# Changfei-Fu/RUMI-SLAM

Measured on AMD Instinct MI355X. Metric: frames/sec ORB extract+match, higher is better.
Workload: dtype u8; 1 GPU; ORB extract (640x480, 8-level pyramid, 1000 features/frame) + brute-force 256-bit Hamming match of consecutive frames (BASELINE.json configs[1]+[2]); scaling=n/a (one GPU), exchange=none

## Files before the change

### rumi_slam_amd/csrc/orb_kernels.hip

```cpp
#include <hip/hip_runtime.h>

#include "orb_device.h"
#include "orb_math.h"

namespace rumi {

struct PatternF { float v[256 * 4]; };
constexpr PatternF make_pattern_f() {
    constexpr int8_t src[256 * 4] = {
#include "orb_pattern.inc"
    };
    PatternF p{};
    for (int i = 0; i < 256 * 4; i++) p.v[i] = (float)src[i];
    return p;
}
__constant__ PatternF c_patternF = make_pattern_f();

__device__ __forceinline__ unsigned xcd_swizzle(unsigned lin, unsigned total) {
    const unsigned q = total >> 3, r = total & 7, xcd = lin & 7;
    return (xcd < r ? xcd * (q + 1) : r * (q + 1) + (xcd - r) * q) + (lin >> 3);
}

struct __attribute__((packed)) U32 { uint32_t v; };
struct __attribute__((packed)) U64 { uint64_t v; };
// ... 367 lines not shown
    const uint32_t to = (g[1] | g[2]) & (g[5] | g[6]), uo = (g[3] | g[4]) & (g[7] | g[0]);
    return (te | ue) & (to | uo);
}
__device__ __forceinline__ uint32_t fast_bytes_ringmask(uint32_t y, uint32_t z) {
    const uint32_t f = ((y & 0x80808080u) | (~(z >> 1) & 0x40404040u));
    return f * 0x41041u;
}

template <int CTP>
__device__ __forceinline__ int fast_score_cell_bytes(const uint8_t *tile, uint8_t *sc, uint16_t *cl, uint16_t *sl, int tp, int dw, int dh, int tlow, int lane) {
    const int TP = CTP ? CTP : tp;
    const int ng = (dw + 7) >> 3;
    const int nItems = ng * dh;
    const unsigned Mng = magic_of(ng);
    const int scDelta = -2 * TP - 3;
    const uint32_t mLast = 0xFFFFu >> (2 * (8 * ng - dw));
    const uint32_t TT = (uint32_t)tlow * 0x01000100u;
    uint32_t *cl32 = reinterpret_cast<uint32_t *>(cl);
    int pending = 0, nScored = 0;
    auto drain = [&]() {
        int head = 0;
        while (pending >= 128) {
            wave_lds_fence();
            fast_score_batch<CTP>(tile, sc, sl, nScored, cl + head, 128, tp, scDelta, tlow, lane);
            head += 128;
            pending -= 128;
        }
        if (head) {
            wave_lds_fence();
            const uint32_t q = cl32[(head >> 1) + lane];
            wave_lds_fence();
            if (2 * lane < pending) cl32[lane] = q;
        }
    };
    for (int base = 0; base < nItems; base += 64) {
        const int ip = base + lane;
        const bool live = ip < nItems;
        const int row = live ? magic_div(ip, Mng) : 0, gi = live ? ip - mul24(row, ng) : 0;
        const int A = mul24(row + 3, TP) + 8 * gi + 4;
        const uint8_t *t = tile + A;
#define RUMI_DW(off) (*reinterpret_cast<const uint32_t *>(t + (off)))
        const uint32_t M3a = RUMI_DW(-3 * TP), M3b = RUMI_DW(-3 * TP + 4), P3a = RUMI_DW(3 * TP), P3b = RUMI_DW(3 * TP + 4);
        const uint32_t M2l = RUMI_DW(-2 * TP - 4), M2a = RUMI_DW(-2 * TP), M2b = RUMI_DW(-2 * TP + 4), M2r = RUMI_DW(-2 * TP + 8);
        const uint32_t P2l = RUMI_DW(2 * TP - 4), P2a = RUMI_DW(2 * TP), P2b = RUMI_DW(2 * TP + 4), P2r = RUMI_DW(2 * TP + 8);
        const uint32_t Cl = RUMI_DW(-4), Ca = RUMI_DW(0), Cb = RUMI_DW(4), Cr = RUMI_DW(8);
#undef RUMI_DW
        const uint32_t m0 = __builtin_amdgcn_alignbyte(M2a, M2l, 2), m1 = __builtin_amdgcn_alignbyte(M2b, M2a, 2), m2 = __builtin_amdgcn_alignbyte(M2r, M2b, 2);
        const uint32_t p0 = __builtin_amdgcn_alignbyte(P2a, P2l, 2), p1 = __builtin_amdgcn_alignbyte(P2b, P2a, 2), p2 = __builtin_amdgcn_alignbyte(P2r, P2b, 2);
        const uint32_t ra[8] = {P3a, p1, __builtin_amdgcn_alignbyte(Cb, Ca, 3), m1, M3a, m0, __builtin_amdgcn_alignbyte(Ca, Cl, 1), p0};
        const uint32_t rb[8] = {P3b, p2, __builtin_amdgcn_alignbyte(Cr, Cb, 3), m2, M3b, m1, __builtin_amdgcn_alignbyte(Cb, Ca, 1), p1};
        uint32_t nba, nda, nbb, ndb;
        fast_bytes_thresholds(Ca, TT, nba, nda);
        fast_bytes_thresholds(Cb, TT, nbb, ndb);
        uint32_t ba[8], ga[8], bb[8], gb[8];
#pragma unroll
        for (int k = 0; k < 8; k++) {
            ba[k] = __builtin_amdgcn_lerp(ra[k], nba, 0u);
            ga[k] = __builtin_amdgcn_lerp(ra[k], nda, 0x01010101u);
            bb[k] = __builtin_amdgcn_lerp(rb[k], nbb, 0u);
            gb[k] = __builtin_amdgcn_lerp(rb[k], ndb, 0x01010101u);
        }
        uint32_t m = __builtin_amdgcn_perm(fast_bytes_ringmask(four_of_eight(bb), four_of_eight_dual(gb)),
                                           fast_bytes_ringmask(four_of_eight(ba), four_of_eight_dual(ga)), 0x0c0c0703u);
        if (gi == ng - 1) m &= mLast;
        if (!live) m = 0;
        if (__ballot(m != 0) != 0) {
            const int cnt = __popc(m);
            const int incl = wave_incl_scan(cnt);
            const int total = __builtin_amdgcn_readlane(incl, 63);
            auto append = [&](uint16_t *w) {
                for (uint32_t r = m; r; r &= r - 1) {
                    const uint32_t b = __builtin_ctz(r);
                    *w++ = (uint16_t)(((uint32_t)A + (b >> 1)) | ((b & 1u) << 15));
                }
            };
            if (pending + total <= kRingCap) {
                append(cl + pending + incl - cnt);
                pending = __builtin_amdgcn_readfirstlane(pending + total);
                drain();
            } else {
                const int half = __builtin_amdgcn_readlane(incl, 31);
                if (lane < 32) append(cl + pending + incl - cnt);
                pending = __builtin_amdgcn_readfirstlane(pending + half);
                drain();
                if (lane >= 32) append(cl + pending + incl - half - cnt);
                pending = __builtin_amdgcn_readfirstlane(pending + total - half);
                drain();
            }
        }
    }
    wave_lds_fence();
    if (pending) fast_score_batch<CTP>(tile, sc, sl, nScored, cl, pending, tp, scDelta, tlow, lane);
    return nScored;
}

struct FastCell {
    const uint8_t *img;
    long long cellIdx;
    int pitch, rows, cols, nd;
    int ox, oy;
    bool live;
};
__device__ __forceinline__ FastCell fast_cell_geom(const DevParams *__restrict__ P, const ImgSrc &src, int cell, int frame, int32_t *__restrict__ cellCnt, int lane) {
    FastCell g;
    g.live = false;
    if (cell >= P->totalCells) return g;
    int level = 0;
    for (int l = 1; l < P->nlevels; l++)
        if (cell >= P->lv[l].cellBase) level = l;
    const DevLevel &L = P->lv[level];
    const int ci = cell - L.cellBase;
    const int ci_i = ci / L.nCols, ci_j = ci - ci_i * L.nCols;
    g.cellIdx = (long long)frame * P->totalCells + cell;
    const int iniY = kBorder + ci_i * L.hCell, iniX = kBorder + ci_j * L.wCell;
    const int maxY = min(iniY + L.hCell + 6, L.maxBY), maxX = min(iniX + L.wCell + 6, L.maxBX);
    g.cols = maxX - iniX; g.rows = maxY - iniY;
    if (iniY >= L.maxBY - 3 || iniX >= L.maxBX - 6 || g.cols < 7 || g.rows < 7) {
        if (lane == 0) cellCnt[g.cellIdx] = 0;
        return g;
    }
    g.img = level_base(src, P, level, frame, &g.pitch) + (long long)iniY * g.pitch + (iniX - 1);
    g.nd = ((g.cols - 6 + 3) >> 2) + 2;
    g.ox = ci_j * L.wCell; g.oy = ci_i * L.hCell;
    g.live = true;
    return g;
}
constexpr int kStageDepth = 10;
template <int TPC>
__device__ __forceinline__ void fast_cell_stage(const FastCell &g, uint8_t *tile, int tp, int lane) {
    const int TP = TPC ? TPC : tp;
    const int ndT = TP >> 2, rps = min(64 / ndT, 7);
    const int r0 = lane / ndT, c = lane - r0 * ndT;
    if (r0 < rps && c < g.nd) {
        const uint8_t *src = g.img + r0 * g.pitch + 4 * c;
        uint8_t *dst = tile + r0 * TP + 4 * c;
        const int nb = (g.rows + rps - 1) / rps, lastRow = g.rows - rps;
        uint32_t v[kStageDepth];
#pragma unroll
        for (int j = 0; j < kStageDepth; j++)
            if (j < nb) v[j] = reinterpret_cast<const U32 *>(src + (long long)min(j * rps, lastRow) * g.pitch)->v;
#pragma unroll
        for (int j = 0; j < kStageDepth; j++)
            if (j < nb) *reinterpret_cast<uint32_t *>(dst + min(j * rps, lastRow) * TP) = v[j];
        for (int j = kStageDepth; j < nb; j++)
            *reinterpret_cast<uint32_t *>(dst + min(j * rps, lastRow) * TP) = reinterpret_cast<const U32 *>(src + (long long)min(j * rps, lastRow) * g.pitch)->v;
    }
}

template <int TPC>
__device__ __forceinline__ void fast_cell_process(const DevParams *__restrict__ P, const FastLds &F, const FastCell &g, uint8_t *tile, uint8_t *sc,
                                                  uint32_t *__restrict__ cellBuf, int32_t *__restrict__ cellCnt, int lane) {
    const int TP = TPC ? TPC : F.tp;
    const int dw = g.cols - 6, dh = g.rows - 6;
    const unsigned Mdw = magic_of(dw), Mtp = magic_of(TP);
    for (int idx = lane * 16; idx < (dh + 2) * TP; idx += 1024) *reinterpret_cast<uint4 *>(&sc[idx]) = make_uint4(0, 0, 0, 0);
    wave_lds_fence();
    const int npx = dw * dh;
    const int scDelta = -2 * TP - 3;
    uint16_t *cl = reinterpret_cast<uint16_t *>(sc + F.scBytes);
    uint16_t *sl = cl + kRingCap;
    int thr = max(1, P->iniTh);
    uint32_t *out = cellBuf + g.cellIdx * P->maxCellCand;
    int found;
#pragma nounroll
    for (int pass = 0;; pass++) {
        const int nScored = fast_score_cell_bytes<TPC>(tile, sc, cl, sl, TP, dw, dh, thr, lane);
        wave_lds_fence();
        const bool listed = nScored <= kScoredCap;
        const int nItems = listed ? nScored : npx;
        found = 0;
        for (int base = 0; base < nItems; base += 128) {
            int si[2];
            bool in[2];
#pragma unroll
            for (int h = 0; h < 2; h++) {
                const int k = base + 64 * h + lane;
                in[h] = k < nItems;
                if (listed) {
                    si[h] = (int)sl[in[h] ? k : 0] + scDelta;
                } else {
                    const int kk = in[h] ? k : 0, py = magic_div(kk, Mdw);
                    si[h] = mul24(py + 1, TP) + (kk - mul24(py, dw)) + 1;
                }
            }
            int v[2];
            bool isMax[2];
#pragma unroll
            for (int h = 0; h < 2; h++) {
                const uint8_t *s = &sc[si[h]];
                v[h] = s[0];
                const int n0 = s[-TP - 1], n1 = s[-TP], n2 = s[-TP + 1], n3 = s[-1], n4 = s[1], n5 = s[TP - 1], n6 = s[TP], n7 = s[TP + 1];
                isMax[h] = in[h] & (v[h] > 0) & (v[h] > n0) & (v[h] > n1) & (v[h] > n2) & (v[h] > n3) & (v[h] > n4) & (v[h] > n5) & (v[h] > n6) & (v[h] > n7);
            }
            const unsigned long long b0 = __ballot(isMax[0]), b1 = __ballot(isMax[1]);
            const int c0 = __popcll(b0);
#pragma unroll
            for (int h = 0; h < 2; h++) {
                if (isMax[h]) {
                    const unsigned long long b = h ? b1 : b0;
                    const int slot = __builtin_amdgcn_mbcnt_hi((uint32_t)(b >> 32), __builtin_amdgcn_mbcnt_lo((uint32_t)b, found + (h ? c0 : 0)));
                    const int py1 = magic_div(si[h], Mtp), px1 = si[h] - mul24(py1, TP);
                    const uint32_t x = (uint32_t)(px1 + 2 + g.ox), y = (uint32_t)(py1 + 2 + g.oy);
                    out[slot] = x | (y << 12) | ((uint32_t)v[h] << 24);
                }
            }
            found += c0 + __popcll(b1);
        }
        if (found > 0 || pass == 1) break;
        thr = max(1, P->minTh);
    }
    if (lane == 0) cellCnt[g.cellIdx] = found;
}

template <int TPC>
__device__ __forceinline__ void fast_cells_body(const DevParams *__restrict__ P, const ImgSrc &src, const FastLds &F, uint32_t *__restrict__ cellBuf,
                                                int32_t *__restrict__ cellCnt, unsigned bx, unsigned gx) {
    extern __shared__ __attribute__((aligned(16))) uint8_t fl[];
    const int lane = threadIdx.x & 63, wave = __builtin_amdgcn_readfirstlane(threadIdx.x >> 6);
    const unsigned wg = xcd_swizzle(blockIdx.y * gx + bx, gx * gridDim.y);
    const int wpg = blockDim.x >> 6;
    const int cell = (wg % gx) * wpg + wave, frame = wg / gx;
    uint8_t *tile = fl + (size_t)wave * F.perWave;
    uint8_t *sc = tile + F.tileBytes;
    const int TP = TPC ? TPC : F.tp;
    const FastCell gA = fast_cell_geom(P, src, cell, frame, cellCnt, lane);
    if (!gA.live) return;
    fast_cell_stage<TPC>(gA, tile, TP, lane);
    fast_cell_process<TPC>(P, F, gA, tile, sc, cellBuf, cellCnt, lane);
}
template <int TPC>
__global__ __launch_bounds__(256) void k_fast_cells(const DevParams *__restrict__ P, ImgSrc src, FastLds F,
                                                    uint32_t *__restrict__ cellBuf, int32_t *__restrict__ cellCnt) {
    fast_cells_body<TPC>(P, src, F, cellBuf, cellCnt, blockIdx.x, gridDim.x);
}

constexpr int kCompactThreads = 256;
__global__ __launch_bounds__(kCompactThreads) void k_compact(const DevParams *__restrict__ P, const uint32_t *__restrict__ cellBuf,
                                                 const int32_t *__restrict__ cellCnt, uint32_t *__restrict__ cand,
                                                 int32_t *__restrict__ levelStart, int32_t *__restrict__ errFlag) {
    extern __shared__ int sStart[];
    __shared__ int part[kCompactThreads];
    const int tid = threadIdx.x, frame = blockIdx.x;
    const int nc = P->totalCells;
    const int32_t *cnt = cellCnt + (long long)frame * nc;
    const int chunk = (nc + kCompactThreads - 1) / kCompactThreads;
    int sum = 0;
    for (int k = 0; k < chunk; k++) {
        const int c = tid * chunk + k;
        if (c < nc) sum += cnt[c];
    }
    const int lane = tid & 63, wave = __builtin_amdgcn_readfirstlane(tid >> 6);
    int inc = sum;
#pragma unroll
    for (int o = 1; o < 64; o <<= 1) {
        const int t = __shfl_up(inc, o);
        if (lane >= o) inc += t;
    }
    if (lane == 63) part[wave] = inc;
    __syncthreads();
    int base = 0, total = 0;
#pragma unroll
    for (int w = 0; w < kCompactThreads / 64; w++) {
        const int t = part[w];
        if (w < wave) base += t;
        total += t;
    }
    if (tid == 0) sStart[nc] = total;
    int run = base + inc - sum;
    for (int k = 0; k < chunk; k++) {
        const int c = tid * chunk + k;
        if (c < nc) { sStart[c] = run; run += cnt[c]; }
    }
    __syncthreads();
    int32_t *ls = levelStart + (long long)frame * (kMaxLevels + 1);
    if (blockIdx.y == 0 && tid <= P->nlevels) {
        const int c = tid < P->nlevels ? P->lv[tid].cellBase : nc;
        ls[tid] = sStart[c];
    }
    if (blockIdx.y == 0 && tid < P->nlevels) {
        const int c0 = P->lv[tid].cellBase, c1 = c0 + P->lv[tid].nCells;
        if (sStart[c1] - sStart[c0] > P->lv[tid].candCap) atomicOr(errFlag, 16);
    }
    uint32_t *out = cand + (long long)frame * P->totalCand;
    const int nOut = min(sStart[nc], P->totalCand);
    const uint32_t *inBase = cellBuf + (long long)frame * nc * P->maxCellCand;
    for (int j = blockIdx.y * kCompactThreads + tid; j < nOut; j += kCompactThreads * gridDim.y) {
        int lo = 0, hi = nc;
        while (hi - lo > 1) {
            const int mid = (lo + hi) >> 1;
            if (sStart[mid] <= j) lo = mid; else hi = mid;
        }
        out[j] = inBase[(long long)lo * P->maxCellCand + (j - sStart[lo])];
    }
}

constexpr int kBlurRowsSmall = 16, kBlurRowsBatch = 64;

struct BlurGrid { int base[kMaxLevels + 1]; int gx[kMaxLevels]; int bw[kMaxLevels]; };
__device__ __forceinline__ uint32_t mad_u24(uint32_t a, uint32_t b, uint32_t c) {
    uint32_t r;
    asm("v_mad_u32_u24 %0, %1, %2, %3" : "=v"(r) : "v"(a), "v"(b), "v"(c));
    return r;
}
template <int VARIANT, int kBlurRows>
__device__ __forceinline__ void blur_body(const DevParams *__restrict__ P, const ImgSrc &src, const BlurGrid &G, unsigned bxg, unsigned gxg) {
    constexpr uint32_t kT2 = VARIANT ? 49u : 48u, kT3 = VARIANT ? 55u : 56u;
    const int lane = threadIdx.x & 63, wave = __builtin_amdgcn_readfirstlane(threadIdx.x >> 6);
    const unsigned wg = xcd_swizzle(blockIdx.y * gxg + bxg, gxg * gridDim.y);
    const int frame = wg / gxg, lin = wg % gxg;
    int level = 0;
    for (int l = 1; l < P->nlevels; l++)
        if (lin >= G.base[l]) level = l;
    const DevLevel &L = P->lv[level];
    const int bx = (lin - G.base[level]) % G.gx[level], by = (lin - G.base[level]) / G.gx[level];
    const int bw = G.bw[level];
    const int xa = bx * bw + lane * 4;
    const int y0 = (by * 4 + wave) * kBlurRows;
    if (y0 >= L.h) return;
    int pitch;
    const uint8_t *img = level_base(src, P, level, frame, &pitch);
    uint8_t *out = src.blur + (long long)frame * P->arenaStride + L.off;
    const int w = L.w, h = L.h;
    const int xLast = (w - 1) & ~3;
    const int xl = min(xa, xLast);
    const bool firstBlock = bx == 0;
    const bool edgeWave = bx * bw + bw + 4 > w;
    const bool produce = lane * 4 < bw && xa < w;
    uint32_t selA = 0x03020100u, selB = 0x07060504u;
    if (edgeWave && xa + 3 >= w && xa <= xLast + 4) {
#pragma unroll
        for (int i = 0; i < 4; i++) {
            const int x = xa + i;
            if (x < w) continue;
            const int sx = 2 * (w - 1) - x, d = (xa - (sx & ~3)) >> 2;
            const uint32_t a = (d == 1 ? 4u : 0u) + (uint32_t)(sx & 3);
            const uint32_t b = d == 0 ? 4u + (uint32_t)(sx & 3) : (uint32_t)i;
            selA = (selA & ~(0xFFu << (8 * i))) | (a << (8 * i));
            selB = (selB & ~(0xFFu << (8 * i))) | (b << (8 * i));
        }
    }
    int ring[7][4];
#pragma unroll
    for (int k = 0; k < 7; k++)
#pragma unroll
        for (int i = 0; i < 4; i++) ring[k][i] = 0;
    const int yEnd = min(y0 + kBlurRows, h), rEnd = yEnd + 3;
    uint8_t *orow = out + (long long)(y0 - 6) * L.pitch + xa - L.pitch;
    const int haloOff = lane == 0 ? (firstBlock ? 0 : -4) : (lane == 63 && !edgeWave && bw == 256 ? 4 : 0);
    uint32_t Cn[7], Hn[7];
    auto fetch = [&](int r, uint32_t &C, uint32_t &H) {
        const int rc = min(r, rEnd - 1);
        const int rr = rc < 0 ? -rc : (rc >= h ? 2 * (h - 1) - rc : rc);
        const uint8_t *row = img + (long long)rr * pitch + xl;
        C = *reinterpret_cast<const uint32_t *>(row);
        H = 0;
        if (haloOff) H = *reinterpret_cast<const uint32_t *>(row + haloOff);
    };
#pragma unroll
    for (int j = 0; j < 7; j++) fetch(y0 - 3 + j, Cn[j], Hn[j]);
    uint32_t Cm[7], Hm[7];
    auto walk7 = [&](const uint32_t (&Cc)[7], const uint32_t (&Hc)[7], int r0) {
#pragma unroll
        for (int j = 0; j < 7; j++) {
            const int r = r0 + j;
            if (r >= rEnd) break;
            orow += L.pitch;
            uint32_t C = Cc[j];
            if (edgeWave) {
                const uint32_t c1 = __shfl_up(C, 1), c2 = __shfl_up(c1, 1);
                C = __builtin_amdgcn_perm(C, __builtin_amdgcn_perm(c1, c2, selA), selB);
            }
            uint32_t Lw = __shfl_up(C, 1), Rw = __shfl_down(C, 1);
            if (lane == 0) Lw = firstBlock ? __builtin_amdgcn_perm(C, C, 0x01020300u) : Hc[j];
            if (lane == 63 && !edgeWave && bw == 256) Rw = Hc[j];
            constexpr uint32_t tA = 18u | (34u << 8) | (kT2 << 16) | (kT3 << 24), tB = kT2 | (34u << 8) | (18u << 16);
            const uint32_t A0 = __builtin_amdgcn_alignbyte(C, Lw, 1), A1 = __builtin_amdgcn_alignbyte(C, Lw, 2), A2 = __builtin_amdgcn_alignbyte(C, Lw, 3);
            const uint32_t B0 = __builtin_amdgcn_alignbyte(Rw, C, 1), B1 = __builtin_amdgcn_alignbyte(Rw, C, 2), B2 = __builtin_amdgcn_alignbyte(Rw, C, 3);
            ring[j][0] = (int)__builtin_amdgcn_udot4(B0, tB, __builtin_amdgcn_udot4(A0, tA, 0u, false), false);
            ring[j][1] = (int)__builtin_amdgcn_udot4(B1, tB, __builtin_amdgcn_udot4(A1, tA, 0u, false), false);
            ring[j][2] = (int)__builtin_amdgcn_udot4(B2, tB, __builtin_amdgcn_udot4(A2, tA, 0u, false), false);
            ring[j][3] = (int)__builtin_amdgcn_udot4(Rw, tB, __builtin_amdgcn_udot4(C, tA, 0u, false), false);
            const int y = r - 3;
            if (y >= y0 && produce) {
                uint32_t o[4];
#pragma unroll
                for (int i = 0; i < 4; i++) {
                    uint32_t acc = mad_u24(kT3, (uint32_t)ring[(j + 4) % 7][i], 32768u);
                    acc = mad_u24(kT2, (uint32_t)(ring[(j + 3) % 7][i] + ring[(j + 5) % 7][i]), acc);
                    acc = mad_u24(34u, (uint32_t)(ring[(j + 2) % 7][i] + ring[(j + 6) % 7][i]), acc);
                    acc = mad_u24(18u, (uint32_t)(ring[(j + 1) % 7][i] + ring[j][i]), acc);
                    if (VARIANT) acc = min(acc, 0x00FFFFFFu);
                    o[i] = acc;
                }
                const uint32_t p01 = __builtin_amdgcn_perm(o[1], o[0], 0x0c0c0602u), p23 = __builtin_amdgcn_perm(o[3], o[2], 0x06020c0cu);
                *reinterpret_cast<uint32_t *>(orow) = p01 | p23;
            }
        }
    };
    for (int r0 = y0 - 3; r0 < rEnd; r0 += 7) {
#pragma unroll
        for (int j = 0; j < 7; j++) Cm[j] = Cn[j], Hm[j] = Hn[j];
        if (r0 + 7 < rEnd) {
#pragma unroll
            for (int j = 0; j < 7; j++) fetch(r0 + 7 + j, Cn[j], Hn[j]);
        }
        walk7(Cm, Hm, r0);
    }
}
template <int VARIANT, int kBlurRows>
__global__ __launch_bounds__(256) void k_blur(const DevParams *__restrict__ P, ImgSrc src, BlurGrid G) {
    blur_body<VARIANT, kBlurRows>(P, src, G, blockIdx.x, gridDim.x);
}
template <int TPC, int VARIANT>
__global__ __launch_bounds__(256) void k_fast_blur(const DevParams *__restrict__ P, ImgSrc src, FastLds F, uint32_t *__restrict__ cellBuf,
                                                   int32_t *__restrict__ cellCnt, BlurGrid G, unsigned gxFast) {
    if (blockIdx.x < gxFast) fast_cells_body<TPC>(P, src, F, cellBuf, cellCnt, blockIdx.x, gxFast);
    else blur_body<VARIANT, kBlurRowsSmall>(P, src, G, blockIdx.x - gxFast, gridDim.x - gxFast);
}

__device__ __forceinline__ int half_wave_sum(int v) {
    v += __builtin_amdgcn_update_dpp(0, v, 0x111, 0xF, 0xF, false);
    v += __builtin_amdgcn_update_dpp(0, v, 0x112, 0xF, 0xF, false);
    v += __builtin_amdgcn_update_dpp(0, v, 0x114, 0xF, 0xF, false);
    v += __builtin_amdgcn_update_dpp(0, v, 0x118, 0xF, 0xF, false);
    v += __builtin_amdgcn_update_dpp(0, v, 0x142, 0xA, 0xF, false);
    const int lo = __builtin_amdgcn_readlane(v, 31), hi = __builtin_amdgcn_readlane(v, 63);
    return (threadIdx.x & 32) ? hi : lo;
}
__device__ __forceinline__ int wave_sum(int v) {
#pragma unroll
    for (int o = 32; o > 0; o >>= 1) v += __shfl_xor(v, o);
    return v;
}

constexpr int kDiscP = 48, kPatchP = 48;
constexpr int kKpPerWg = 8;

struct AssembleArgs {
    const uint32_t *selLevel; const int32_t *selLevelCnt; int selLevelCap, lap0, lap1;
    int32_t *counts; long long countsStride; int32_t *errFlag, *errMirror;
    uint32_t *selPackedOut, *selMetaOut; int32_t *selCountOut;
};
template <int kKpGroups, bool kAssemble>
__global__ __launch_bounds__(256, 7) void k_orient_desc(const DevParams *__restrict__ P, ImgSrc src,
                                                     const uint32_t *__restrict__ selPacked,
                                                     const uint32_t *__restrict__ selMeta,
                                                     const int32_t *__restrict__ selCount, int selCap,
                                                     RumiKeyPoint *__restrict__ kpOut, long long kpStride, uint8_t *__restrict__ descOut,
                                                     long long descStride, int outCap, AssembleArgs A) {
    static_assert(kDiscP == kPatchP, "the disc and the patch share their rows");
    __shared__ __attribute__((aligned(16))) uint8_t sWin[kKpPerWg][37 * kPatchP];
    __shared__ __attribute__((aligned(16))) float sPat[256 * 4];
    __shared__ int4 sLv[kMaxLevels];
    __shared__ float2 sLvF[kMaxLevels];
    reinterpret_cast<float4 *>(sPat)[threadIdx.x] = reinterpret_cast<const float4 *>(c_patternF.v)[threadIdx.x];
    if (threadIdx.x < (unsigned)P->nlevels) {
        const DevLevel &Lv = P->lv[threadIdx.x];
        sLv[threadIdx.x] = threadIdx.x == 0 ? make_int4(0, src.l0Pitch, (int)Lv.off, Lv.pitch) : make_int4((int)Lv.off, Lv.pitch, (int)Lv.off, Lv.pitch);
        sLvF[threadIdx.x] = make_float2(Lv.scale, Lv.patchSize);
    }
    const int lane = threadIdx.x & 31, hw = threadIdx.x >> 5;
    const unsigned wg = xcd_swizzle(blockIdx.y * gridDim.x + blockIdx.x, gridDim.x * gridDim.y);
    const int kb = (wg % gridDim.x) * (kKpPerWg * kKpGroups) + hw, frame = wg / gridDim.x;
    int cnt;
    __shared__ uint32_t sOwnPk[kAssemble ? kKpPerWg * kKpGroups : 1], sOwnMt[kAssemble ? kKpPerWg * kKpGroups : 1];
    if constexpr (!kAssemble) {
        cnt = selCount[frame];
        __syncthreads();
    } else {
        __shared__ int sLvStart[kMaxLevels + 1], sRed[2], sOwnF[kKpPerWg * kKpGroups];
        const int nl = P->nlevels, tid = threadIdx.x;
        if (tid == 0) {
            int run = 0;
            for (int l = 0; l < nl; l++) { sLvStart[l] = run; run += A.selLevelCnt[(long long)frame * nl + l]; }
            sLvStart[nl] = run; sRed[0] = 0; sRed[1] = 0;
        }
        __syncthreads();
        const int total = sLvStart[nl], kbase = (wg % gridDim.x) * (kKpPerWg * kKpGroups);
        const bool first = wg % gridDim.x == 0, over = total > selCap;
        int32_t *counts = reinterpret_cast<int32_t *>(reinterpret_cast<uint8_t *>(A.counts) + frame * A.countsStride);
        if (over) {
            if (first && tid == 0) { A.selCountOut[frame] = 0; counts[0] = total; counts[1] = 0; const int old = atomicOr(A.errFlag, 8); if (A.errMirror) *A.errMirror = old | 8; }
            return;
        }
        cnt = total;
        auto key_at = [&](int k, int *levelOut) -> uint32_t {
            int level = 0;
            while (k >= sLvStart[level + 1]) level++;
            *levelOut = level;
            return A.selLevel[((long long)frame * nl + level) * A.selLevelCap + (k - sLvStart[level])];
        };
        auto lapped = [&](uint32_t pk, int level) -> bool {
            float x = (float)((int)(pk & 0xFFF) + kBorder);
            if (level != 0) x = x * P->lv[level].scale;
            return x >= (float)A.lap0 && x <= (float)A.lap1;
        };
        int before = 0, all = 0;
        for (int k = tid; k < total; k += 256) {
            int level;
            const uint32_t pk = key_at(k, &level);
            const int f = lapped(pk, level) ? 1 : 0;
            all += f; before += k < kbase ? f : 0;
        }
#pragma unroll
        for (int o = 32; o > 0; o >>= 1) { before += __shfl_xor(before, o); all += __shfl_xor(all, o); }
        if ((tid & 63) == 0) { atomicAdd(&sRed[0], before); atomicAdd(&sRed[1], all); }
        if (tid < kKpPerWg * kKpGroups) {
            const int k = kbase + tid;
            int level = 0;
            uint32_t pk = 0;
            int f = 0;
            if (k < total) { pk = key_at(k, &level); f = lapped(pk, level) ? 1 : 0; }
            sOwnPk[tid] = pk; sOwnMt[tid] = (uint32_t)level; sOwnF[tid] = f;
        }
        __syncthreads();
        if (tid == 0) {
            int b = sRed[0];
            for (int j = 0; j < kKpPerWg * kKpGroups; j++) {
                const int k = kbase + j;
                if (k >= total) break;
                const int f = sOwnF[j], slot = f ? (total - 1 - b) : (k - b);
                b += f;
                sOwnMt[j] |= (uint32_t)slot << 8;
            }
            if (first) {
                counts[0] = total; counts[1] = total - sRed[1];
                A.selCountOut[frame] = total;
                if (A.errMirror) *A.errMirror = *A.errFlag;
            }
        }
        __syncthreads();
        if (tid < kKpPerWg * kKpGroups && kbase + tid < total) {
            A.selPackedOut[(long long)frame * selCap + kbase + tid] = sOwnPk[tid];
            A.selMetaOut[(long long)frame * selCap + kbase + tid] = sOwnMt[tid];
        }
    }
#ifdef RUMI_OD_STAMP
    long long st[8] = {0, 0, 0, 0, 0, 0, 0, 0}, stLast = clock64();
#define OD_STAMP(k) do { const long long t_ = clock64(); st[k] += t_ - stLast; stLast = t_; } while (0)
#else
#define OD_STAMP(k) do { } while (0)
#endif

    struct __attribute__((packed, aligned(4))) Q16 { uint32_t x, y, z, w; };
    struct __attribute__((packed, aligned(4))) Q8 { uint32_t x, y; };
    auto ld16 = [](const uint8_t *q) { const Q16 t = *reinterpret_cast<const Q16 *>(q); return make_uint4(t.x, t.y, t.z, t.w); };
    auto ld8 = [](const uint8_t *q) { const Q8 t = *reinterpret_cast<const Q8 *>(q); return make_uint2(t.x, t.y); };
    struct Staged { uint4 d0, d1, p0, p1, q0, q1; uint2 p2, q2; uint32_t d2; };
    const bool dRow = lane < 31, qRow = lane < 5;
    const uint8_t *frame0 = src.l0 + (long long)frame * src.l0FrameStride, *framePyr = src.pyr + (long long)frame * P->arenaStride,
                  *frameBlur = src.blur + (long long)frame * P->arenaStride;
    auto fetch_disc = [&](uint32_t pk, uint32_t meta, bool live, Staged &S) {
        if (!live || !dRow) return;
        const int level = meta & 0xFF, x = (int)(pk & 0xFFF) + kBorder, y = (int)((pk >> 12) & 0xFFF) + kBorder;
        const int4 lv = sLv[level];
        const uint8_t *cr = (level == 0 ? frame0 : framePyr) + (lv.x + (y - kHalfPatch + lane) * lv.y + ((x - kHalfPatch) & ~3));
        S.d0 = ld16(cr); S.d1 = ld16(cr + 16); S.d2 = *reinterpret_cast<const uint32_t *>(cr + 32);
    };
    auto fetch_patch = [&](uint32_t pk, uint32_t meta, bool live, Staged &S) {
        if (!live) return;
        const int level = meta & 0xFF, x = (int)(pk & 0xFFF) + kBorder, y = (int)((pk >> 12) & 0xFFF) + kBorder;
        const int4 lv = sLv[level];
        const uint8_t *br = frameBlur + (lv.z + (y - 18 + lane) * lv.w + ((x - 18) & ~3)), *br2 = br + 32 * lv.w;
        S.p0 = ld16(br); S.p1 = ld16(br + 16); S.p2 = ld8(br + 32);
        if (qRow) { S.q0 = ld16(br2); S.q1 = ld16(br2 + 16); S.q2 = ld8(br2 + 32); }
    };
    auto stage_disc = [&](bool live, const Staged &S) {
        if (!live || !dRow) return;
        uint8_t *dst = &sWin[hw][lane * kDiscP];
        *reinterpret_cast<uint4 *>(dst) = S.d0; *reinterpret_cast<uint4 *>(dst + 16) = S.d1; *reinterpret_cast<uint32_t *>(dst + 32) = S.d2;
    };
    auto stage_patch = [&](bool live, const Staged &S) {
        if (!live) return;
        {
            uint8_t *dst = &sWin[hw][lane * kPatchP];
            *reinterpret_cast<uint4 *>(dst) = S.p0; *reinterpret_cast<uint4 *>(dst + 16) = S.p1; *reinterpret_cast<uint2 *>(dst + 32) = S.p2;
        }
        if (qRow) {
            uint8_t *dst = &sWin[hw][(lane + 32) * kPatchP];
            *reinterpret_cast<uint4 *>(dst) = S.q0; *reinterpret_cast<uint4 *>(dst + 16) = S.q1; *reinterpret_cast<uint2 *>(dst + 32) = S.q2;
        }
    };
    auto orientation = [&](uint32_t pk) -> float {
        const int x = (int)(pk & 0xFFF) + kBorder;
        const int xd = (x - kHalfPatch) & ~3;
        const uint8_t *dc = &sWin[hw][kHalfPatch * kDiscP + (x - xd)];
        const int u = lane - kHalfPatch;
        const int vmaxU = lane < 31 ? P->umax[u < 0 ? -u : u] : -1;
        const int mid = dc[u];
        int colSum = vmaxU >= 0 ? mid : 0, m01 = 0;
#pragma unroll
        for (int v = 1; v <= kHalfPatch; v++) {
            const int lo = dc[-v * kDiscP + u], hi = dc[v * kDiscP + u];
            const bool in = v <= vmaxU;
            colSum += in ? lo + hi : 0;
            m01 += in ? v * (hi - lo) : 0;
        }
        int m10 = u * colSum;
        m10 = half_wave_sum(m10);
        m01 = half_wave_sum(m01);
        OD_STAMP(4);
        return fast_atan2_deg((float)m01, (float)m10);
    };
    auto describe = [&](uint32_t pk, uint32_t meta, float angle) {
        const int level = meta & 0xFF, slot = (int)(meta >> 8);
        const int x = (int)(pk & 0xFFF) + kBorder, y = (int)((pk >> 12) & 0xFFF) + kBorder, score = (int)(pk >> 24);
        const int xp = (x - 18) & ~3;
        const float factorPI = (float)(3.1415926535897932384626433832795 / 180.f);
        const float ang = angle * factorPI;
        const float a = cosf_glibc(ang), b = sinf_glibc(ang);
        const uint8_t *bc = &sWin[hw][18 * kPatchP + (x - xp)];
        uint32_t w = 0;
        OD_STAMP(5);
#pragma unroll
        for (int j = 0; j < 8; j++) {
            const float4 pt = reinterpret_cast<const float4 *>(sPat)[j * 32 + lane];
            const float x0 = pt.x, y0 = pt.y, x1 = pt.z, y1 = pt.w;
            const int r0 = cv_round_f(x0 * b + y0 * a), c0 = cv_round_f(x0 * a - y0 * b);
            const int r1 = cv_round_f(x1 * b + y1 * a), c1 = cv_round_f(x1 * a - y1 * b);
            const int t0 = bc[r0 * kPatchP + c0], t1 = bc[r1 * kPatchP + c1];
            const unsigned long long bal = __ballot(t0 < t1);
            const uint32_t lo = (uint32_t)bal, hi = (uint32_t)(bal >> 32);
            asm("s_nop 4\n\tv_writelane_b32 %0, %1, %3\n\tv_writelane_b32 %0, %2, %4" : "+v"(w) : "s"(lo), "s"(hi), "n"(j), "n"(32 + j));
        }
        OD_STAMP(6);
        if (slot < outCap) {
            if (lane < 8) reinterpret_cast<uint32_t *>(descOut + frame * descStride + (long long)slot * 32)[lane] = w;
            if (lane == 0) {
                RumiKeyPoint kp;
                kp.x = (float)x; kp.y = (float)y;
                const float2 lf = sLvF[level];
                if (level != 0) { kp.x = kp.x * lf.x; kp.y = kp.y * lf.x; }
                kp.size = lf.y;
                kp.angle = angle;
                kp.response = (float)score;
                kp.octave = level;
                kp.class_id = -1;
                reinterpret_cast<RumiKeyPoint *>(reinterpret_cast<uint8_t *>(kpOut) + frame * kpStride)[slot] = kp;
            }
        }
    };

    const uint32_t *selP = selPacked + (long long)frame * selCap, *selM = selMeta + (long long)frame * selCap;
    auto key_rec = [&](int k, uint32_t &pk, uint32_t &mt) {
        if constexpr (kAssemble) { const int j = k - (kb - hw); pk = sOwnPk[j]; mt = sOwnMt[j]; }
        else { pk = selP[k]; mt = selM[k]; }
    };
    bool liveC = kb < cnt, liveN = kb + kKpPerWg < cnt;
    uint32_t pkC = 0, mtC = 0, pkN = 0, mtN = 0;
    if (liveC) key_rec(kb, pkC, mtC);
    if (liveN && kKpGroups > 1) key_rec(kb + kKpPerWg, pkN, mtN);
    if (kKpGroups == 1) liveN = false;
    Staged S;
    fetch_disc(pkC, mtC, liveC, S);
    fetch_patch(pkC, mtC, liveC, S);
#pragma unroll
    for (int g = 0; g < kKpGroups; g++) {
        if (!__any(liveC)) break;
        OD_STAMP(0);
        stage_disc(liveC, S);
        OD_STAMP(1);
        const int k2 = kb + (g + 2) * kKpPerWg;
        const bool liveNN = g + 2 < kKpGroups && k2 < cnt;
        uint32_t pkNN = 0, mtNN = 0;
        if (liveNN) key_rec(k2, pkNN, mtNN);
        if (g + 1 < kKpGroups) fetch_disc(pkN, mtN, liveN, S);
        OD_STAMP(2);
        float angle = 0.f;
        if (liveC) angle = orientation(pkC);
        stage_patch(liveC, S);
        if (g + 1 < kKpGroups) fetch_patch(pkN, mtN, liveN, S);
        if (liveC) describe(pkC, mtC, angle);
        OD_STAMP(3);
        pkC = pkN; mtC = mtN; liveC = liveN;
        pkN = pkNN; mtN = mtNN; liveN = liveNN;
    }
#ifdef RUMI_OD_STAMP
    if (threadIdx.x == 0 && (blockIdx.x % 8) == 0 && blockIdx.y == 0) printf("od wg %d: loop-head %lld stage(wait loads) %lld issue-next %lld | IC_Angle %lld trig %lld rBRIEF %lld store %lld\n", (int)blockIdx.x, st[0], st[1], st[2], st[4], st[5], st[6], st[3]);
#endif
}

void launch_resize(const DevParams *dP, const DevParams &hP, ImgSrc src, const int16_t *coef, const RowTap *rowTab, int level, int nframes,
                   hipStream_t st, int32_t *clearWord) {
    const int rows = hP.lv[level].h >= 200 ? 8 : 4;
    dim3 g((hP.lv[level].w + 255) / 256, (hP.lv[level].h + 4 * rows - 1) / (4 * rows), nframes);
    if (rows == 8) hipLaunchKernelGGL(k_resize<8>, g, dim3(256), 0, st, dP, src, coef, rowTab, level, clearWord);
    else hipLaunchKernelGGL(k_resize<4>, g, dim3(256), 0, st, dP, src, coef, rowTab, level, clearWord);
}
void launch_pyramid_tiles(const DevParams *dP, ImgSrc src, const int16_t *coef, const RowTap *rowTab, const PyrTile *tiles, int ntiles, int bufBytes,
                          int tabEntries, int nframes, hipStream_t st, int32_t *clearWord) {
    hipLaunchKernelGGL(k_pyramid_tiles, dim3(ntiles, nframes), dim3(256), (size_t)2 * bufBytes + (size_t)tabEntries * 8, st, dP, src, coef, rowTab, tiles, bufBytes, clearWord);
}
static FastLds fast_lds_of(const DevParams &hP) {
// ... 108 lines not shown
```

Before: 286,600 frames/s.

## Use DPP lane shifts and packed dot2 vertical taps in the Gaussian blur

Replaces the __shfl_up/__shfl_down cross-lane moves in the blur with wave-wide DPP row shifts, folding the halo and mirror selection into perm selectors. The horizontal pass is rewritten with per-output dot4 weight vectors. Pairs of consecutive horizontal row sums are packed into 16-bit halves so the vertical 7-tap pass uses three udot2 ops plus one mad instead of four mads and three adds. The halo load now runs unconditionally, and the packing assumes the horizontal sums fit in 16 bits.

New measurement: 289,500 frames/s (median of 6 runs). +1.0%, better.

```diff
diff --git a/rumi_slam_amd/csrc/orb_kernels.hip b/rumi_slam_amd/csrc/orb_kernels.hip
--- a/rumi_slam_amd/csrc/orb_kernels.hip
+++ b/rumi_slam_amd/csrc/orb_kernels.hip
@@ -693,6 +693,8 @@
     asm("v_mad_u32_u24 %0, %1, %2, %3" : "=v"(r) : "v"(a), "v"(b), "v"(c));
     return r;
 }
+__device__ __forceinline__ uint32_t dpp_wave_shr1(uint32_t old, uint32_t v) { return (uint32_t)__builtin_amdgcn_update_dpp((int)old, (int)v, 0x138, 0xf, 0xf, false); }
+__device__ __forceinline__ uint32_t dpp_wave_shl1(uint32_t old, uint32_t v) { return (uint32_t)__builtin_amdgcn_update_dpp((int)old, (int)v, 0x130, 0xf, 0xf, false); }
 template <int VARIANT, int kBlurRows>
 __device__ __forceinline__ void blur_body(const DevParams *__restrict__ P, const ImgSrc &src, const BlurGrid &G, unsigned bxg, unsigned gxg) {
     constexpr uint32_t kT2 = VARIANT ? 49u : 48u, kT3 = VARIANT ? 55u : 56u;
@@ -730,11 +732,12 @@
             selB = (selB & ~(0xFFu << (8 * i))) | (b << (8 * i));
         }
     }
-    int ring[7][4];
+    uint32_t ring[7][4], rPrev[4] = {0, 0, 0, 0};
 #pragma unroll
     for (int k = 0; k < 7; k++)
 #pragma unroll
         for (int i = 0; i < 4; i++) ring[k][i] = 0;
+    const uint32_t selL = firstBlock && lane == 0 ? 0x01020300u : 0x07060504u;
     const int yEnd = min(y0 + kBlurRows, h), rEnd = yEnd + 3;
     uint8_t *orow = out + (long long)(y0 - 6) * L.pitch + xa - L.pitch;
     const int haloOff = lane == 0 ? (firstBlock ? 0 : -4) : (lane == 63 && !edgeWave && bw == 256 ? 4 : 0);
@@ -744,8 +747,7 @@
         const int rr = rc < 0 ? -rc : (rc >= h ? 2 * (h - 1) - rc : rc);
         const uint8_t *row = img + (long long)rr * pitch + xl;
         C = *reinterpret_cast<const uint32_t *>(row);
-        H = 0;
-        if (haloOff) H = *reinterpret_cast<const uint32_t *>(row + haloOff);
+        H = *reinterpret_cast<const uint32_t *>(row + haloOff);
     };
 #pragma unroll
     for (int j = 0; j < 7; j++) fetch(y0 - 3 + j, Cn[j], Hn[j]);
@@ -756,30 +758,41 @@
             const int r = r0 + j;
             if (r >= rEnd) break;
             orow += L.pitch;
-            uint32_t C = Cc[j];
+            uint32_t C = Cc[j], Ro = Hc[j];
             if (edgeWave) {
-                const uint32_t c1 = __shfl_up(C, 1), c2 = __shfl_up(c1, 1);
+                const uint32_t c1 = dpp_wave_shr1(C, C), c2 = dpp_wave_shr1(c1, c1);
                 C = __builtin_amdgcn_perm(C, __builtin_amdgcn_perm(c1, c2, selA), selB);
-            }
-            uint32_t Lw = __shfl_up(C, 1), Rw = __shfl_down(C, 1);
-            if (lane == 0) Lw = firstBlock ? __builtin_amdgcn_perm(C, C, 0x01020300u) : Hc[j];
-            if (lane == 63 && !edgeWave && bw == 256) Rw = Hc[j];
-            constexpr uint32_t tA = 18u | (34u << 8) | (kT2 << 16) | (kT3 << 24), tB = kT2 | (34u << 8) | (18u << 16);
-            const uint32_t A0 = __builtin_amdgcn_alignbyte(C, Lw, 1), A1 = __builtin_amdgcn_alignbyte(C, Lw, 2), A2 = __builtin_amdgcn_alignbyte(C, Lw, 3);
-            const uint32_t B0 = __builtin_amdgcn_alignbyte(Rw, C, 1), B1 = __builtin_amdgcn_alignbyte(Rw, C, 2), B2 = __builtin_amdgcn_alignbyte(Rw, C, 3);
-            ring[j][0] = (int)__builtin_amdgcn_udot4(B0, tB, __builtin_amdgcn_udot4(A0, tA, 0u, false), false);
-            ring[j][1] = (int)__builtin_amdgcn_udot4(B1, tB, __builtin_amdgcn_udot4(A1, tA, 0u, false), false);
-            ring[j][2] = (int)__builtin_amdgcn_udot4(B2, tB, __builtin_amdgcn_udot4(A2, tA, 0u, false), false);
-            ring[j][3] = (int)__builtin_amdgcn_udot4(Rw, tB, __builtin_amdgcn_udot4(C, tA, 0u, false), false);
+                Ro = C;
+            }
+            const uint32_t Lw = dpp_wave_shr1(__builtin_amdgcn_perm(Hc[j], C, selL), C), Rw = dpp_wave_shl1(Ro, C);
+            constexpr uint32_t k0 = 18u, k1 = 34u, k2 = kT2, k3 = kT3;
+            constexpr uint32_t w0L = (k0 << 8) | (k1 << 16) | (k2 << 24), w0C = k3 | (k2 << 8) | (k1 << 16) | (k0 << 24);
+            constexpr uint32_t w1L = (k0 << 16) | (k1 << 24), w1C = k2 | (k3 << 8) | (k2 << 16) | (k1 << 24), w1R = k0;
+            constexpr uint32_t w2L = k0 << 24, w2C = k1 | (k2 << 8) | (k3 << 16) | (k2 << 24), w2R = k1 | (k0 << 8);
+            constexpr uint32_t w3C = k0 | (k1 << 8) | (k2 << 16) | (k3 << 24), w3R = k2 | (k1 << 8) | (k0 << 16);
+            uint32_t rCur[4];
+            rCur[0] = __builtin_amdgcn_udot4(C, w0C, __builtin_amdgcn_udot4(Lw, w0L, 0u, false), false);
+            rCur[1] = __builtin_amdgcn_udot4(Rw, w1R, __builtin_amdgcn_udot4(C, w1C, __builtin_amdgcn_udot4(Lw, w1L, 0u, false), false), false);
+            rCur[2] = __builtin_amdgcn_udot4(Rw, w2R, __builtin_amdgcn_udot4(C, w2C, __builtin_amdgcn_udot4(Lw, w2L, 0u, false), false), false);
+            rCur[3] = __builtin_amdgcn_udot4(Rw, w3R, __builtin_amdgcn_udot4(C, w3C, 0u, false), false);
+#pragma unroll
+            for (int i = 0; i < 4; i++) {
+                ring[(j + 6) % 7][i] = rPrev[i] | (rCur[i] << 16);
+                rPrev[i] = rCur[i];
+            }
             const int y = r - 3;
             if (y >= y0 && produce) {
+                typedef unsigned short v2u16 __attribute__((ext_vector_type(2)));
+                auto dot2 = [](uint32_t q, uint32_t taps, uint32_t acc) {
+                    return __builtin_amdgcn_udot2(__builtin_bit_cast(v2u16, q), __builtin_bit_cast(v2u16, taps), acc, false);
+                };
                 uint32_t o[4];
 #pragma unroll
                 for (int i = 0; i < 4; i++) {
-                    uint32_t acc = mad_u24(kT3, (uint32_t)ring[(j + 4) % 7][i], 32768u);
-                    acc = mad_u24(kT2, (uint32_t)(ring[(j + 3) % 7][i] + ring[(j + 5) % 7][i]), acc);
-                    acc = mad_u24(34u, (uint32_t)(ring[(j + 2) % 7][i] + ring[(j + 6) % 7][i]), acc);
-                    acc = mad_u24(18u, (uint32_t)(ring[(j + 1) % 7][i] + ring[j][i]), acc);
+                    uint32_t acc = dot2(ring[(j + 1) % 7][i], 18u | (34u << 16), 32768u);
+                    acc = dot2(ring[(j + 3) % 7][i], kT2 | (kT3 << 16), acc);
+                    acc = dot2(ring[(j + 5) % 7][i], kT2 | (34u << 16), acc);
+                    acc = mad_u24(18u, rCur[i], acc);
                     if (VARIANT) acc = min(acc, 0x00FFFFFFu);
                     o[i] = acc;
                 }
```
